# nintendops/EPN_PointCloud

Measured on AMD Instinct MI355X. Metric: point-clouds/sec fwd+bwd, ModelNet40 N=1024 A=60, higher is better.
Workload: dtype f32

## Files before the change

epn_pointcloud_amd/csrc/c_api.hip:

```cpp
#include <atomic>
#include <cstdlib>
#include <cstring>
#include <cxxabi.h>

#include "conv_internal.h"

using namespace epn;

static std::atomic<int> g_policy{0};
static bool force_generic() { return g_policy.load(std::memory_order_relaxed) == 1; }

namespace epn {
bool first_layer_on_valu() { return g_policy.load(std::memory_order_relaxed) == 2; }
#ifdef EPN_TUNING
int kernel_policy() { return g_policy.load(std::memory_order_relaxed); }
#else
int kernel_policy() { return 0; }
#endif
}

namespace {
thread_local const void *t_stub = nullptr;
thread_local bool t_stub_aux = true;
}
namespace epn {
void note_kernel(const void *host_stub, bool aux) {
    if (aux && t_stub) return;
    t_stub = host_stub;
    t_stub_aux = aux;
}
}

extern "C" const char *epn_last_kernel(void) {
    static thread_local char out[320];
    out[0] = 0;
    const void *stub = t_stub;
    t_stub = nullptr;
    t_stub_aux = true;
    if (!stub) return out;
    const char *mangled = hipKernelNameRefByPtr(stub, nullptr);
    if (!mangled) return out;
    int status = 0;
    char *dem = abi::__cxa_demangle(mangled, nullptr, nullptr, &status);
    const char *b = (status == 0 && dem) ? dem : mangled;
    if (!std::strncmp(b, "void ", 5)) b += 5;
    static const char anon[] = "(anonymous namespace)::";
    size_t o = 0;
    int depth = 0;
    for (size_t i = 0; b[i] && o + 1 < sizeof(out);) {
        if (!std::strncmp(b + i, anon, sizeof(anon) - 1)) { i += sizeof(anon) - 1; continue; }
        if (b[i] == '<') ++depth;
        else if (b[i] == '>') --depth;
        else if (b[i] == '(' && depth == 0) break;
        out[o++] = b[i++];
    }
    out[o] = 0;
    std::free(dem);
    return out;
}

extern "C" int epn_set_kernel_policy(int policy) {
#ifdef EPN_TUNING
    if (policy != 0 && policy != 1 && policy != 2 && (policy & ~0xff) != 0x100 && (policy & ~0xff) != 0x200 && (policy & ~0xff) != 0x400 && (policy & ~0xff) != 0x800 && (policy & ~0xff) != 0x900) return EPN_EINVAL;
#else
    if (policy != 0 && policy != 1 && policy != 2) return EPN_EINVAL;
#endif
    g_policy.store(policy, std::memory_order_relaxed);
    return 0;
}

static int check_desc(const epn_inter_desc *d) {
    if (!d) return EPN_ENULL;
    if (d->b < 0 || d->p1 < 1 || d->p2 < 0 || d->nn < 1 || d->na < 1 || d->ks < 1 || d->cin < 1 || d->cout < 1)
        return EPN_EINVAL;
    if (d->ks > EPN_KS_GENERIC_MAX) return EPN_EINVAL;
    if (!(d->sigma > 0.f) && !d->dense_w) return EPN_EINVAL;
    if (!d->ball_idx) return EPN_ENULL;
    if (!d->dense_w && (!d->xyz || !d->new_xyz || !d->anchors || !d->kernels)) return EPN_ENULL;
    return 0;
}

static bool use_mfma(const epn_inter_desc *d) { return inter_uses_mfma(d) && !force_generic() && !d->dense_w; }

extern "C" const char *epn_version(void) { return "epn_so3conv 0.5 (gfx950)"; }
extern "C" int epn_abi_version(void) { return EPN_ABI_VERSION; }

extern "C" const char *epn_strerror(int code) {
    switch (code) {
        case 0: return "success";
        case EPN_EINVAL: return "epn: invalid size or unsupported shape";
        case EPN_EWORKSPACE: return "epn: workspace missing or too small";
        case EPN_ENULL: return "epn: required pointer is NULL";
        default: return code > 0 ? hipGetErrorString((hipError_t)code) : "epn: unknown error";
    }
}

extern "C" int epn_inter_is_fused(const epn_inter_desc *d) {
    return d && (use_mfma(d) || (inter_c1_fwd_ok(d) && !force_generic())) ? 1 : 0;
}

extern "C" int epn_intra_is_fused(int na, int kn, int cin, int cout) {
    return intra_uses_mfma(na, kn, cin, cout) && !force_generic() ? 1 : 0;
}

extern "C" size_t epn_inter_workspace_bytes(const epn_inter_desc *d) {
    if (!d) return 0;
    InterWs w = inter_ws(d);
    if (force_generic() || d->dense_w) {
        epn_inter_desc g = *d;
        g.cin = d->cin; g.cout = d->cout;
        const size_t big = (size_t)d->b * d->p2 * d->na * d->cin * d->ks;
        return (w.big_off + rnd64(big)) * sizeof(float);
    }
    return w.total_floats * sizeof(float);
}

static int prep(const epn_inter_desc *d, void *workspace, size_t bytes, bool need_big, InterWs &ws, float *&base,
                hipStream_t st, bool need_rk = true) {
    int rc = check_desc(d);
    if (rc) return rc;
    ws = inter_ws(d);
    const size_t big = need_big ? rnd64((size_t)d->b * d->p2 * d->na * d->cin * d->ks)
                                : ws.total_floats - ws.big_off;
    if (!workspace || bytes < (ws.big_off + big) * sizeof(float)) return EPN_EWORKSPACE;
    base = static_cast<float *>(workspace);
    if (!d->dense_w && need_rk) {
        rc = launch_rk_table(d, base + ws.rk_off, st);
        if (rc) return rc;
    }
    return 0;
}

extern "C" int epn_inter_weights_f32(const epn_inter_desc *d, float *w, epn_stream_t stream) {
    int rc = check_desc(d);
    if (rc) return rc;
    if (!w || !d->xyz || !d->new_xyz || !d->anchors || !d->kernels) return EPN_ENULL;
    if (d->b == 0 || d->p2 == 0) return 0;
    return launch_inter_weights(d, w, epn_stream(stream));
}

extern "C" int epn_inter_so3conv_fwd_f32(const epn_inter_desc *d, const float *feats_cl, const float *W,
                                         float *out_cl, void *workspace, size_t workspace_bytes,
                                         epn_stream_t stream) {
    hipStream_t st = epn_stream(stream);
    InterWs ws;
    float *base = nullptr;
    const bool mf = d && use_mfma(d);
    int rc = prep(d, workspace, workspace_bytes, !mf, ws, base, st, !mf);
// ... 431 lines not shown
```

epn_pointcloud_amd/csrc/gemm.h:

```cpp
#pragma once
#include "epn_common.h"

namespace epn {

constexpr int GEMM_MAX_PROB = 6;

struct GemmNtProb {
    const void *A, *Bt;
    void *C;
    long long M, lda, ldb, ldc;
    int N, K;
    int tiles_n;
    unsigned tile0;
    unsigned ntile;
    const void *Bp;
    float *stats;
    const float *a_amax, *b_amax;
    unsigned *c_amax;
};
struct GemmNtBatch {
    int nprob;
    unsigned ntiles;
    GemmNtProb p[GEMM_MAX_PROB];
};
// ... 131 lines not shown
    mfma_term(acc, al, bh);
    mfma_term(acc, am, bm);
    mfma_term(acc, ah, bm);
    mfma_term(acc, am, bh);
    mfma_term(acc, ah, bh);
}
template <int TM, int TN>
__device__ __forceinline__ void f2_terms(gemm_f32x16 (&acc)[TM][TN], const gemm_f16x8 (&ah)[TM], const gemm_f16x8 (&al)[TM],
                                         const gemm_f16x8 (&bh)[TN], const gemm_f16x8 (&bl)[TN]) {
    mfma_term(acc, ah, bl);
    mfma_term(acc, al, bh);
    mfma_term(acc, ah, bh);
}
template <int TM, int TN>
__device__ __forceinline__ float f2_unscale(gemm_f32x16 (&acc)[TM][TN], float ux, float uy) {
    float chk = 0.0f;
#pragma unroll
    for (int i = 0; i < TM; ++i)
#pragma unroll
        for (int j = 0; j < TN; ++j)
#pragma unroll
            for (int r = 0; r < 16; ++r) {
                chk = fmaf(acc[i][j][r], 0.0f, chk);
                acc[i][j][r] = acc[i][j][r] * ux * uy;
            }
    return chk;
}

template <int TM, int TN, typename TO>
__device__ __forceinline__ void nt_col_stats(const gemm_f32x16 (&acc)[TM][TN], float *__restrict__ part, long long M, int N,
                                             long long row0, int col0, int li, int lj) {
#pragma unroll
    for (int i = 0; i < TM; ++i) {
        const long long rb = row0 + 32 * i;
        if (rb >= M) continue;
#pragma unroll
        for (int j = 0; j < TN; ++j) {
            float s1 = 0.f, s2 = 0.f;
#pragma unroll
            for (int r = 0; r < 16; ++r) {
                float v = acc[i][j][r];
                if constexpr (sizeof(TO) == 2) v = (float)(__bf16)v;
                s1 += v;
                s2 = fmaf(v, v, s2);
            }
            s1 += __shfl_xor(s1, 32, 64);
            s2 += __shfl_xor(s2, 32, 64);
            const int n = col0 + 32 * j + li;
            if (lj == 0 && n < N) {
                float2 *o = reinterpret_cast<float2 *>(part + (((size_t)(rb >> 5)) * N + n) * 2);
                *o = make_float2(s1, s2);
            }
        }
    }
}
#endif

#ifdef __HIPCC__
template <int TM, int TN, typename TO>
__device__ __forceinline__ void nt_c_amax(const gemm_f32x16 (&acc)[TM][TN], unsigned *__restrict__ out) {
    float mf = 0.0f;
#pragma unroll
    for (int i = 0; i < TM; ++i)
#pragma unroll
        for (int j = 0; j < TN; ++j)
#pragma unroll
            for (int r = 0; r < 16; r += 2) mf = fmaxf(fmaxf(mf, fabsf(acc[i][j][r])), fabsf(acc[i][j][r + 1]));
    if constexpr (sizeof(TO) == 2) mf = (float)(__bf16)mf;
    unsigned m = __builtin_bit_cast(unsigned, mf);
    m = m < 0x7f800000u ? m : 0u;
#pragma unroll
    for (int o = 32; o >= 1; o >>= 1) {
        const unsigned v = (unsigned)__shfl_xor((int)m, o, 64);
        m = v > m ? v : m;
    }
    if ((threadIdx.x & 63) == 0 && m > __atomic_load_n(out, __ATOMIC_RELAXED)) atomicMax(out, m);
}
#endif

long long f2_nonfinite_take_gemm(bool reset);
long long f2_nonfinite_take_x3(bool reset);
long long f2_nonfinite_take_bwd(bool reset);

int kernel_policy();

int launch_gemm_nt(GemmNtBatch &B, int dtype, int out_dtype, hipStream_t st);
bool gemm_nt_x3_ok(const GemmNtBatch &B);
size_t gemm_nt_x3_workspace(const GemmNtBatch &B);
int launch_gemm_nt_x3(GemmNtBatch &B, void *ws, size_t ws_bytes, hipStream_t st, int npl = 3);
size_t gemm_nt_f2_workspace(const GemmNtBatch &B);
int launch_absmax(const float *src, long long ld, long long rows, long long cols, float *out, hipStream_t st);
int launch_scale_scalar(float *v, float factor, hipStream_t st, unsigned tag = 0);
int launch_absmax_unless_tagged(const float *src, long long n, float *slot, unsigned tag, hipStream_t st);
int launch_gemm_tn(GemmTnArgs &G, int dtype, hipStream_t st);
int launch_gemm_tn_batch(GemmTnBatch &B, int dtype, void *ws, size_t ws_bytes, hipStream_t st);
size_t gemm_tn_batch_workspace(GemmTnBatch &B, int dtype);
void gemm_tn_tile(int dtype, int N1, int N2, int *bn1, int *bn2);
int gemm_tn_splits(int dtype, long long R, int N1, int N2);
int launch_transpose_cast(const void *src, void *dst, int rows, int cols, int src_bf16, int dst_bf16, hipStream_t st);
int launch_cast(const void *src, void *dst, size_t n, int src_bf16, int dst_bf16, hipStream_t st);
int launch_cast_add(const float *src, const void *add_bf16, void *dst_bf16, size_t n, hipStream_t st);

}
```

epn_pointcloud_amd/csrc/gemm_tn.hip:

```cpp
#include "conv_internal.h"
#include "gemm.h"

namespace epn {
namespace {
EPN_F2_SENTINEL_DECL


#ifndef EPN_TN_GROUP_TARGET_BF16
#define EPN_TN_GROUP_TARGET_BF16 768
#endif
#ifndef EPN_TN_GROUP_TARGET_F32
#define EPN_TN_GROUP_TARGET_F32 1024
#endif
#ifndef EPN_TN_SINGLE_TARGET_BF16
#define EPN_TN_SINGLE_TARGET_BF16 512
#endif
#ifndef EPN_TN_SWZ
#define EPN_TN_SWZ 1
#endif
__device__ __forceinline__ int tn_row_swz(int r) { return 2 * ((r & 3) | (((r >> 3) & 1) << 2)); }
template <bool SWZ>
__device__ __forceinline__ int tn_swz_col(int col, int r) {
    if constexpr (!SWZ) return col;
    return (((col >> 3) ^ tn_row_swz(r)) << 3) | (col & 7);
}
#ifndef EPN_TN_WIDE_NSTG
#define EPN_TN_WIDE_NSTG 3
#endif
#ifndef EPN_TN_NARROW_NSTG
#define EPN_TN_NARROW_NSTG 4
#endif
#ifndef EPN_TN_NARROW_STAGE_KB
#define EPN_TN_NARROW_STAGE_KB 32
#endif
constexpr int tn_ring_kr(int wgm, int wgn, int tm, int tn) {
    const int step_b = 32 * 2 * 16 * (wgm * tm + wgn * tn);
    int kr = 1;
    while (2 * kr * step_b <= EPN_TN_NARROW_STAGE_KB * 1024 && 2 * kr * step_b * EPN_TN_NARROW_NSTG <= 160 * 1024) kr *= 2;
    return kr;
}
#ifndef EPN_TN_NARROW_WGS
#define EPN_TN_NARROW_WGS 1
#endif
__device__ __forceinline__ unsigned tn_tile_of(unsigned lb, unsigned ntiles, unsigned nsplit) {
    return epn_xcd_tile(lb, (ntiles * nsplit + 7u) & ~7u);
}

template <int W, int K>
__device__ __forceinline__ void tn_frag_k(const char *p, float (&v)[W][K], int k) {
    static_assert(W == 1 || W == 2 || W == 4, "fragment width");
    if constexpr (W == 4) {
        const f32x4 q = *reinterpret_cast<const f32x4 *>(p);
        v[0][k] = q[0]; v[1][k] = q[1]; v[2][k] = q[2]; v[3][k] = q[3];
    } else if constexpr (W == 2) {
        const f32x2 q = *reinterpret_cast<const f32x2 *>(p);
        v[0][k] = q[0]; v[1][k] = q[1];
    } else {
        v[0][k] = *reinterpret_cast<const float *>(p);
    }
}
template <int W>
__device__ __forceinline__ void tn_frag(const char *p, float (&v)[W]) {
    static_assert(W == 1 || W == 2 || W == 4, "fragment width");
    if constexpr (W == 4) {
        const f32x4 q = *reinterpret_cast<const f32x4 *>(p);
        v[0] = q[0]; v[1] = q[1]; v[2] = q[2]; v[3] = q[3];
    } else if constexpr (W == 2) {
        const f32x2 q = *reinterpret_cast<const f32x2 *>(p);
        v[0] = q[0]; v[1] = q[1];
    } else {
        v[0] = *reinterpret_cast<const float *>(p);
    }
}

template <int WGM, int WGN, int TM, int TN, int BR, int X3 = 0>
__global__ __launch_bounds__(64 * WGM * WGN) void gemm_tn_f32_kernel(GemmTnBatch B) {
    constexpr int NW = WGM * WGN;
    constexpr int BN1 = WGM * TM * 32, BN2 = WGN * TN * 32;
    constexpr int ROWF = BN1 + BN2;
    constexpr int STAGE_B = BR * ROWF * 4;
    constexpr int NI = STAGE_B / 1024;
    constexpr int IPW = (NI + NW - 1) / NW;
    static_assert(STAGE_B % 1024 == 0, "stage must be a whole number of 1 KiB pieces");
    __shared__ __attribute__((aligned(1024))) char smem[2 * STAGE_B];

    const int lane = threadIdx.x & 63;
    const int wave = __builtin_amdgcn_readfirstlane(threadIdx.x >> 6);
    int pi = 0;
#pragma unroll
    for (int i = 1; i < GEMM_MAX_PROB; ++i)
        if (i < B.nprob && blockIdx.x >= B.p[i].block0) pi = i;
    const GemmTnArgs &G = B.p[pi];
    const unsigned tile = tn_tile_of(blockIdx.x - G.block0, G.ntiles, (unsigned)G.nsplit) % G.ntiles;
    const unsigned split = tn_tile_of(blockIdx.x - G.block0, G.ntiles, (unsigned)G.nsplit) / G.ntiles;
    if (split >= (unsigned)G.nsplit) return;
    const int n1_0 = (int)(tile / G.tiles_n2) * BN1, n2_0 = (int)(tile % G.tiles_n2) * BN2;
    const long long nchunk = G.R / BR;
    const long long c0 = nchunk * split / G.nsplit, c1 = nchunk * (split + 1) / G.nsplit;
    const int nk = (int)(c1 - c0);
    const float *__restrict__ X = static_cast<const float *>(G.X);
    const float *__restrict__ Y = static_cast<const float *>(G.Y);

    const float *src[IPW];
    long long sstep[IPW];
#pragma unroll
    for (int i = 0; i < IPW; ++i) {
        const int q = wave + i * NW;
        const int fo = 256 * q + 4 * lane;
        const int r = fo / ROWF, c = fo % ROWF;
        if (c < BN1) {
            int n = n1_0 + c;
            n = n < G.N1 - 4 ? n : G.N1 - 4;
            src[i] = X + (c0 * BR + r) * G.ldx + n;
            sstep[i] = (long long)BR * G.ldx;
        } else {
            int n = n2_0 + (c - BN1);
            n = n < G.N2 - 4 ? n : G.N2 - 4;
            src[i] = Y + (c0 * BR + r) * G.ldy + n;
            sstep[i] = (long long)BR * G.ldy;
        }
    }
    auto stage_one = [&](int buf, int i) {
        const int q = wave + i * NW;
// ... 515 lines not shown
            src[i] += sstep[i];
        }
    };

    const int wm = wave / WGN, wn = wave % WGN;
    const int li = lane & 15, lg = lane >> 4;
    const int tr_row = 8 * lg + (li >> 2), tr_col = 4 * (li & 3);

    f32x4 acc[TM][TN];
#pragma unroll
    for (int i = 0; i < TM; ++i)
#pragma unroll
        for (int j = 0; j < TN; ++j) acc[i][j] = f32x4{0.f, 0.f, 0.f, 0.f};

#pragma unroll
    for (int s = 0; s < NSTG - 1; ++s)
        if (s < nst) stage(s);
    typedef short s16x8 __attribute__((ext_vector_type(8)));
    for (int kt = 0; kt < nst; ++kt) {
        const int ahead = nst - 1 - kt;
        if (NSTG == 4 && ahead >= 2) asm volatile("s_waitcnt vmcnt(%0)" ::"n"(2 * IPW) : "memory");
        else if (ahead >= 1) asm volatile("s_waitcnt vmcnt(%0)" ::"n"(IPW) : "memory");
        else asm volatile("s_waitcnt vmcnt(0)" ::: "memory");
        __builtin_amdgcn_s_barrier();
        asm volatile("" ::: "memory");
        const char *sbase = smem + (kt % NSTG) * STAGE_B;
#pragma unroll
        for (int ks = 0; ks < KR; ++ks) {
            if (KR > 1 && kt * KR + ks >= nk) break;
            const char *base = sbase + ks * (32 * ROWE * 2);
            s16x4 lo[TM + TN], hi[TM + TN];
#pragma unroll
            for (int f = 0; f < TM + TN; ++f) {
                const int col = tn_swz_col<SWZ>(f < TN ? BN1 + (wn * TN + f) * 16 + tr_col : (wm * TM + (f - TN)) * 16 + tr_col, tr_row);
                const unsigned ad =
                    (unsigned)(uintptr_t)(__attribute__((address_space(3))) char *)(base + (tr_row * ROWE + col) * 2);
                asm volatile("ds_read_b64_tr_b16 %0, %1" : "=v"(lo[f]) : "v"(ad));
                asm volatile("ds_read_b64_tr_b16 %0, %1 offset:%2" : "=v"(hi[f]) : "v"(ad), "n"(4 * ROWE * 2));
            }
            bf16x8 b[TN];
#pragma unroll
            for (int i = 0; i < TM; ++i) {
                asm volatile("s_waitcnt lgkmcnt(%0)" ::"n"(2 * (TM - 1 - i)) : "memory");
                if (i == 0) {
#pragma unroll
                    for (int j = 0; j < TN; ++j) {
                        asm volatile("" : "+v"(lo[j]), "+v"(hi[j]));
                        const s16x8 v = {lo[j][0], lo[j][1], lo[j][2], lo[j][3], hi[j][0], hi[j][1], hi[j][2], hi[j][3]};
                        b[j] = __builtin_bit_cast(bf16x8, v);
                    }
                }
                asm volatile("" : "+v"(lo[TN + i]), "+v"(hi[TN + i]));
                const s16x8 va = {lo[TN + i][0], lo[TN + i][1], lo[TN + i][2], lo[TN + i][3],
                                  hi[TN + i][0], hi[TN + i][1], hi[TN + i][2], hi[TN + i][3]};
                const bf16x8 a = __builtin_bit_cast(bf16x8, va);
#pragma unroll
                for (int j = 0; j < TN; ++j) {
                    acc[i][j] = __builtin_amdgcn_mfma_f32_16x16x32_bf16(a, b[j], acc[i][j], 0, 0, 0);
                    if (ks == 0 && i == 0 && j == 0) {
                        __builtin_amdgcn_sched_barrier(0);
                        if (kt + NSTG - 1 < nst) stage((kt + NSTG - 1) % NSTG);
                        __builtin_amdgcn_sched_barrier(0);
                    }
                }
            }
        }
    }

    float *__restrict__ C = G.nsplit > 1 ? static_cast<float *>(G.part) + (size_t)split * G.N1 * G.N2
                                         : static_cast<float *>(G.C);
    const long long ldc = G.nsplit > 1 ? G.N2 : G.ldc;
#pragma unroll
    for (int i = 0; i < TM; ++i)
#pragma unroll
        for (int j = 0; j < TN; ++j)
#pragma unroll
            for (int r = 0; r < 4; ++r) {
                const int n1 = n1_0 + (wm * TM + i) * 16 + 4 * lg + r;
                const int n2 = n2_0 + (wn * TN + j) * 16 + li;
                if (n1 < G.N1 && n2 < G.N2) C[(long long)n1 * ldc + n2] = acc[i][j][r];
            }
}

__global__ __launch_bounds__(256) void gemm_tn_reduce_kernel(GemmTnBatch B) {
    const GemmTnArgs &G = B.p[blockIdx.y];
    if (G.nsplit <= 1) return;
    const float *__restrict__ part = static_cast<const float *>(G.part);
    float *__restrict__ C = static_cast<float *>(G.C);
    const size_t n = (size_t)G.N1 * G.N2;
    const size_t stride = (size_t)gridDim.x * blockDim.x;
    if ((G.N2 & 3) == 0 && (G.ldc & 3) == 0 && !((uintptr_t)C & 15)) {
        const size_t n4 = n >> 2;
        for (size_t i = (size_t)blockIdx.x * blockDim.x + threadIdx.x; i < n4; i += stride) {
            const f32x4 *p = reinterpret_cast<const f32x4 *>(part) + i;
            f32x4 a[8];
#pragma unroll
            for (int u = 0; u < 8; ++u) a[u] = f32x4{0.f, 0.f, 0.f, 0.f};
            int k = 0;
            for (; k + 8 <= G.nsplit; k += 8)
#pragma unroll
                for (int u = 0; u < 8; ++u) {
                    const f32x4 v = p[(size_t)(k + u) * n4];
                    a[u][0] += v[0]; a[u][1] += v[1]; a[u][2] += v[2]; a[u][3] += v[3];
                }
            for (; k < G.nsplit; ++k) {
                const f32x4 v = p[(size_t)k * n4];
                a[0][0] += v[0]; a[0][1] += v[1]; a[0][2] += v[2]; a[0][3] += v[3];
            }
            f32x4 r;
#pragma unroll
            for (int e = 0; e < 4; ++e)
                r[e] = ((a[0][e] + a[1][e]) + (a[2][e] + a[3][e])) + ((a[4][e] + a[5][e]) + (a[6][e] + a[7][e]));
            const size_t e0 = i << 2;
            *reinterpret_cast<f32x4 *>(C + (e0 / G.N2) * G.ldc + (e0 % G.N2)) = r;
        }
        return;
    }
    for (size_t i = (size_t)blockIdx.x * blockDim.x + threadIdx.x; i < n; i += stride) {
        float s = 0.f;
        for (int k = 0; k < G.nsplit; ++k) s += part[(size_t)k * n + i];
        C[(i / G.N2) * G.ldc + (i % G.N2)] = s;
    }
}

template <int SP>
__global__ __launch_bounds__(256) void gemm_tn_reduce_sp_kernel(GemmTnBatch B) {
    constexpr int QB = 256 / SP;
    __shared__ f32x4 red[SP][QB];
    const GemmTnArgs &G = B.p[blockIdx.y];
    if (G.nsplit <= 1) return;
    const f32x4 *__restrict__ part = static_cast<const f32x4 *>(G.part);
    float *__restrict__ C = static_cast<float *>(G.C);
    const size_t n4 = ((size_t)G.N1 * G.N2) >> 2;
    const int ql = threadIdx.x % QB, g = threadIdx.x / QB;
    for (size_t q0 = (size_t)blockIdx.x * QB; q0 < n4; q0 += (size_t)gridDim.x * QB) {
        const size_t q = q0 + ql;
        f32x4 a[4];
#pragma unroll
        for (int u = 0; u < 4; ++u) a[u] = f32x4{0.f, 0.f, 0.f, 0.f};
        if (q < n4) {
            int k = g;
            for (; k + 3 * SP < G.nsplit; k += 4 * SP)
#pragma unroll
                for (int u = 0; u < 4; ++u) {
                    const f32x4 v = part[(size_t)(k + u * SP) * n4 + q];
                    a[u][0] += v[0]; a[u][1] += v[1]; a[u][2] += v[2]; a[u][3] += v[3];
                }
            for (; k < G.nsplit; k += SP) {
                const f32x4 v = part[(size_t)k * n4 + q];
                a[0][0] += v[0]; a[0][1] += v[1]; a[0][2] += v[2]; a[0][3] += v[3];
            }
        }
        f32x4 r;
#pragma unroll
        for (int e = 0; e < 4; ++e) r[e] = (a[0][e] + a[1][e]) + (a[2][e] + a[3][e]);
        red[g][ql] = r;
        __syncthreads();
        if (g == 0 && q < n4) {
            for (int j = 1; j < SP; ++j) {
                const f32x4 v = red[j][ql];
                r[0] += v[0]; r[1] += v[1]; r[2] += v[2]; r[3] += v[3];
            }
            const size_t e0 = q << 2;
            *reinterpret_cast<f32x4 *>(C + (e0 / G.N2) * G.ldc + (e0 % G.N2)) = r;
        }
        __syncthreads();
    }
}

template <typename T>
__global__ void gemm_tn_generic_kernel(const T *__restrict__ X, const T *__restrict__ Y, float *__restrict__ C,
                                       long long R, int N1, int N2, long long ldx, long long ldy, long long ldc) {
    const long long i = (long long)blockIdx.x * blockDim.x + threadIdx.x;
    if (i >= (long long)N1 * N2) return;
    const int n1 = (int)(i / N2), n2 = (int)(i % N2);
    float s = 0.f;
    for (long long r = 0; r < R; ++r) s = fmaf((float)X[r * ldx + n1], (float)Y[r * ldy + n2], s);
    C[(long long)n1 * ldc + n2] = s;
}

enum TnFamily { TN_F32, TN_PLANES, TN_BF16, TN_RING };
#define EPN_TN_F32_INSTANCES(X)                                                                                      \
    X(1, 8, 1, 2, 32)                                                                                 \
    X(2, 2, 1, 1, 32)                                                                                 \
    X(2, 2, 1, 2, 32)                                                                                 \
    X(1, 8, 2, 1, 32)                                                                                 \
    X(1, 4, 2, 4, 16)                                                                                 \
    X(2, 2, 2, 1, 32)                                                                                 \
    X(2, 2, 2, 2, 32)                                                                                 \
    X(2, 4, 2, 2, 32)                                                                                 \
    X(1, 8, 4, 2, 32)
#define EPN_TN_PLANES_INSTANCES(X)                                                                                   \
    X(1, 8, 1, 2, 32)                                                                                 \
    X(1, 8, 2, 2, 16)                                                                                 \
    X(2, 4, 2, 2, 32)                                   \
    X(1, 8, 4, 2, 16)                                                                                 \
    X(2, 4, 4, 2, 16)
#define EPN_TN_BF16_INSTANCES(X)                                                                                     \
    X(1, 4, 2, 4)                                                                                     \
    X(1, 4, 4, 4)                                                                                     \
    X(2, 2, 4, 8)
#define EPN_TN_RING_NARROW(X, TM, TN) X(2, 2, TM, TN, EPN_TN_NARROW_NSTG, tn_ring_kr(2, 2, TM, TN))
#define EPN_TN_RING_INSTANCES(X)                                                                                     \
    EPN_TN_RING_NARROW(X, 1, 1)                                                                       \
    EPN_TN_RING_NARROW(X, 2, 1)                                                                       \
    EPN_TN_RING_NARROW(X, 1, 2)                                                                       \
    EPN_TN_RING_NARROW(X, 2, 2)                                                                       \
    EPN_TN_RING_NARROW(X, 4, 2)                                                                       \
    EPN_TN_RING_NARROW(X, 8, 2)                                                                       \
    EPN_TN_RING_NARROW(X, 1, 4)                                                                       \
    EPN_TN_RING_NARROW(X, 2, 4)                                                                       \
    EPN_TN_RING_NARROW(X, 4, 4)                                                                       \
    EPN_TN_RING_NARROW(X, 8, 4)                                                                       \
    X(2, 2, 4, 8, EPN_TN_WIDE_NSTG, 1)

struct TnChoice {
    TnFamily family;
    int bn1, bn2;
    bool planes;
    size_t ws_bytes;
    size_t amax_off;
};

inline bool tn_has_instance(TnFamily f, int bn1, int bn2) {
#define EPN_TN_IS32(WGM, WGN, TM, TN, ...) || (bn1 == WGM * TM * 32 && bn2 == WGN * TN * 32)
#define EPN_TN_IS16(WGM, WGN, TM, TN, ...) || (bn1 == WGM * TM * 16 && bn2 == WGN * TN * 16)
    switch (f) {
        case TN_F32: return false EPN_TN_F32_INSTANCES(EPN_TN_IS32);
        case TN_PLANES: return false EPN_TN_PLANES_INSTANCES(EPN_TN_IS32);
        case TN_BF16: return false EPN_TN_BF16_INSTANCES(EPN_TN_IS16);
        case TN_RING: return false EPN_TN_RING_INSTANCES(EPN_TN_IS16);
    }
#undef EPN_TN_IS32
#undef EPN_TN_IS16
    return false;
}

template <typename T>
int launch_tn_instance(const TnChoice &ch, const GemmTnBatch &B, hipStream_t st, int x3) {
    const dim3 grid(B.nblocks);
#define EPN_TN_F32(WGM, WGN, TM, TN, BR)                                                                                       \
    if (ch.bn1 == WGM * TM * 32 && ch.bn2 == WGN * TN * 32) {                                                                  \
        if (x3 == 3) EPN_LAUNCH((gemm_tn_f32_kernel<WGM, WGN, TM, TN, BR, 3>), grid, dim3(64 * WGM * WGN), 0, st, B);          \
        else if (x3 == 2) EPN_LAUNCH((gemm_tn_f32_kernel<WGM, WGN, TM, TN, BR, 2>), grid, dim3(64 * WGM * WGN), 0, st, B);     \
        else EPN_LAUNCH((gemm_tn_f32_kernel<WGM, WGN, TM, TN, BR, 0>), grid, dim3(64 * WGM * WGN), 0, st, B);                  \
        return 0;                                                                                                              \
    }
#define EPN_TN_PLANES(WGM, WGN, TM, TN, BR)                                                                                    \
    if (ch.bn1 == WGM * TM * 32 && ch.bn2 == WGN * TN * 32) {                                                                  \
        if (x3 == 3) EPN_LAUNCH((gemm_tn_x3_kernel<WGM, WGN, TM, TN, BR, 3>), grid, dim3(64 * WGM * WGN), 0, st, B);           \
        else EPN_LAUNCH((gemm_tn_x3_kernel<WGM, WGN, TM, TN, BR, 2>), grid, dim3(64 * WGM * WGN), 0, st, B);                   \
        return 0;                                                                                                              \
    }
#define EPN_TN_BF16(WGM, WGN, TM, TN)                                                                                          \
    if (ch.bn1 == WGM * TM * 16 && ch.bn2 == WGN * TN * 16) {                                                                  \
        EPN_LAUNCH((gemm_tn_bf16_kernel<WGM, WGN, TM, TN>), grid, dim3(64 * WGM * WGN), 0, st, B);                             \
        return 0;                                                                                                              \
    }
#define EPN_TN_RING(WGM, WGN, TM, TN, NSTG, KR)                                                                                \
    if (ch.bn1 == WGM * TM * 16 && ch.bn2 == WGN * TN * 16) {                                                                  \
        EPN_LAUNCH((gemm_tn_bf16_ring_kernel<WGM, WGN, TM, TN, NSTG, KR>), grid, dim3(64 * WGM * WGN), 0, st, B);              \
        return 0;                                                                                                              \
    }
    if constexpr (sizeof(T) == 4) {
        if (ch.family == TN_F32) { EPN_TN_F32_INSTANCES(EPN_TN_F32) }
        if (ch.family == TN_PLANES) { EPN_TN_PLANES_INSTANCES(EPN_TN_PLANES) }
    } else {
        if (ch.family == TN_BF16) { EPN_TN_BF16_INSTANCES(EPN_TN_BF16) }
        if (ch.family == TN_RING) { EPN_TN_RING_INSTANCES(EPN_TN_RING) }
    }
#undef EPN_TN_F32
#undef EPN_TN_PLANES
#undef EPN_TN_BF16
#undef EPN_TN_RING
    return EPN_EINVAL;
}

#ifndef EPN_TN_GROUP_PLANES
#define EPN_TN_GROUP_PLANES 512
#endif
inline int tn_group_planes(int x3) { return x3 == 2 ? EPN_TN_GROUP_PLANES / 2 : EPN_TN_GROUP_PLANES; }
inline bool tn_planes_form(int nprob, int N2, int x3) { return N2 >= (nprob == 1 ? 512 : tn_group_planes(x3)); }

template <typename T>
bool tn_fast_ok(const GemmTnArgs &G) {
    constexpr int E16 = ElemOf<T>::PER16;
    return G.R > 0 && G.R % 32 == 0 && G.N1 >= E16 && G.N2 >= E16 && G.ldx % E16 == 0 && G.ldy % E16 == 0 &&
           !((uintptr_t)G.X & 15) && !((uintptr_t)G.Y & 15) && G.N1 % E16 == 0 && G.N2 % E16 == 0;
}

template <typename T>
TnChoice tn_plan(GemmTnBatch &B, void *ws, int x3 = 0) {
    const int bf = sizeof(T) == 2 ? 1 : (x3 ? 2 : 0);
    int max1 = 0, min2 = 1 << 30;
    for (int i = 0; i < B.nprob; ++i) {
        max1 = B.p[i].N1 > max1 ? B.p[i].N1 : max1;
        min2 = B.p[i].N2 < min2 ? B.p[i].N2 : min2;
    }
    int bn1, bn2;
    gemm_tn_tile(B.nprob > 1 && bf == 2 ? 0 : bf, max1, B.nprob > 1 && min2 < 256 ? 256 : min2, &bn1, &bn2);
    if (B.nprob > 1 && bf == 2 && min2 >= tn_group_planes(x3)) {
        int min1 = 1 << 30;
        for (int i = 0; i < B.nprob; ++i) min1 = B.p[i].N1 < min1 ? B.p[i].N1 : min1;
        if (min1 >= 256) { bn1 = 256; bn2 = 256; }
    }
    if (B.nprob > 1 && x3 == 2 && min2 < 256) { bn1 = 128; bn2 = 128; }
    long long tiles[GEMM_MAX_PROB], chunks[GEMM_MAX_PROB];
    for (int i = 0; i < B.nprob; ++i) {
        GemmTnArgs &G = B.p[i];
        G.tiles_n2 = (G.N2 + bn2 - 1) / bn2;
        G.ntiles = (unsigned)((G.N1 + bn1 - 1) / bn1) * G.tiles_n2;
        tiles[i] = G.ntiles;
        chunks[i] = G.R / 32;
    }
    if (B.nprob == 1) {
        B.p[0].nsplit = gemm_tn_splits(bf, B.p[0].R, B.p[0].N1, B.p[0].N2);
    } else {
        const long long target = bf == 1 ? EPN_TN_GROUP_TARGET_BF16 : EPN_TN_GROUP_TARGET_F32;
        long long S = 8;
        for (long long cand = 8; cand <= 8192; ++cand) {
            long long blocks = 0;
            for (int i = 0; i < B.nprob; ++i) blocks += tiles[i] * ((chunks[i] + cand - 1) / cand);
            S = cand;
            if (blocks <= target) break;
        }
        for (int i = 0; i < B.nprob; ++i) {
            long long sp = (chunks[i] + S - 1) / S;
            sp = sp < 1 ? 1 : (sp > 512 ? 512 : sp);
            B.p[i].nsplit = (int)sp;
        }
    }
    size_t off = 0;
    unsigned blk = 0;
    for (int i = 0; i < B.nprob; ++i) {
        GemmTnArgs &G = B.p[i];
        G.block0 = blk;
        blk += (G.ntiles * (unsigned)G.nsplit + 7u) & ~7u;
        G.part = nullptr; G.part_bytes = 0;
        if (G.nsplit > 1) {
            const size_t nb = (size_t)G.nsplit * G.N1 * G.N2 * sizeof(float);
            if (ws) G.part = static_cast<char *>(ws) + off;
            G.part_bytes = nb;
            off += (nb + 255) & ~(size_t)255;
        }
    }
    B.nblocks = blk;
    for (int i = 0; i < B.nprob; ++i) B.p[i].Xp = nullptr;
    const bool planes = x3 && tn_has_instance(TN_PLANES, bn1, bn2) && tn_planes_form(B.nprob, min2, x3);
    if (planes)
        for (int i = 0; i < B.nprob; ++i) {
            GemmTnArgs &G = B.p[i];
            G.Xp = ws ? static_cast<char *>(ws) + off : reinterpret_cast<const void *>(1);
            off += ((size_t)2 * x3 * G.R * G.N1 + 255) & ~(size_t)255;
        }
    size_t amax_off = 0;
    if (x3 == 2) {
        amax_off = off;
        off += 256;
    }
    TnFamily family = planes ? TN_PLANES : TN_F32;
    if constexpr (sizeof(T) == 2) family = (B.nprob == 1 ? bn2 <= 128 : bn1 == 128) ? TN_RING : TN_BF16;
    return TnChoice{family, bn1, bn2, planes, off, amax_off};
}

template <typename T>
int launch_tn_typed(GemmTnBatch &B, void *ws, size_t ws_bytes, hipStream_t st, int x3 = 0) {
    bool fast = true;
    for (int i = 0; i < B.nprob; ++i) {
        const GemmTnArgs &G = B.p[i];
        if (G.R < 0 || G.N1 < 1 || G.N2 < 1) return EPN_EINVAL;
        if (!G.C) return EPN_ENULL;
        if (G.R > 0 && (!G.X || !G.Y)) return EPN_ENULL;
        fast = fast && tn_fast_ok<T>(G);
    }
    if (!fast) {
        for (int i = 0; i < B.nprob; ++i) {
            const GemmTnArgs &G = B.p[i];
            const long long n = (long long)G.N1 * G.N2;
            EPN_LAUNCH((gemm_tn_generic_kernel<T>), dim3((unsigned)((n + 255) / 256)), dim3(256), 0, st,
                               static_cast<const T *>(G.X), static_cast<const T *>(G.Y), static_cast<float *>(G.C), G.R,
                               G.N1, G.N2, G.ldx, G.ldy, G.ldc);
            EPN_CHECK_LAUNCH();
        }
        return 0;
    }
    const TnChoice ch = tn_plan<T>(B, ws, x3);
    if (ch.ws_bytes > 0 && (!ws || ws_bytes < ch.ws_bytes)) return EPN_EWORKSPACE;
    if (!tn_has_instance(ch.family, ch.bn1, ch.bn2)) return EPN_EINVAL;
    if constexpr (sizeof(T) == 4) {
        if (x3 == 2) {
            float *slots = reinterpret_cast<float *>(static_cast<char *>(ws) + ch.amax_off);
            for (int i = 0; i < B.nprob; ++i) {
                GemmTnArgs &G = B.p[i];
                if (!G.x_amax) {
                    int rc = launch_absmax(static_cast<const float *>(G.X), G.ldx, G.R, G.N1, slots + 2 * i, st);
                    if (rc) return rc;
                    G.x_amax = slots + 2 * i;
                }
                if (!G.y_amax) {
                    int rc = launch_absmax(static_cast<const float *>(G.Y), G.ldy, G.R, G.N2, slots + 2 * i + 1, st);
                    if (rc) return rc;
                    G.y_amax = slots + 2 * i + 1;
                }
            }
        }
        if (ch.planes) {
            for (int i = 0; i < B.nprob; ++i) {
                const GemmTnArgs &G = B.p[i];
                const long long n = (G.R >> 3) * G.N1;
                if (x3 == 3)
                    EPN_LAUNCH_AUX(split_octets_kernel, dim3((unsigned)((n + 255) / 256)), dim3(256), 0, st,
                                   static_cast<const float *>(G.X), G.ldx, G.R, G.N1, static_cast<u32x4 *>(const_cast<void *>(G.Xp)));
                else
                    EPN_LAUNCH_AUX(split_octets2_kernel, dim3((unsigned)((n + 255) / 256)), dim3(256), 0, st,
                                   static_cast<const float *>(G.X), G.ldx, G.R, G.N1, static_cast<u32x4 *>(const_cast<void *>(G.Xp)), G.x_amax);
                EPN_CHECK_LAUNCH();
            }
        }
    }
    const int rc = launch_tn_instance<T>(ch, B, st, x3);
    if (rc) return rc;
    EPN_CHECK_LAUNCH();
    bool any_split = false;
    size_t nmax = 0;
    for (int i = 0; i < B.nprob; ++i) {
        any_split = any_split || B.p[i].nsplit > 1;
        const size_t n = (size_t)B.p[i].N1 * B.p[i].N2;
        nmax = n > nmax ? n : nmax;
    }
    if (any_split) {
        const size_t nv = (nmax + 3) / 4;
        bool quads = true;
        int smax = 1;
        for (int i = 0; i < B.nprob; ++i) {
            const GemmTnArgs &G = B.p[i];
            quads = quads && (G.N2 & 3) == 0 && (G.ldc & 3) == 0 && !((uintptr_t)G.C & 15);
            smax = G.nsplit > smax ? G.nsplit : smax;
        }
        int sp = 1;
        while (quads && sp < 64 && smax > 16 * sp && nv * B.nprob * sp * 4 <= (1u << 20)) sp *= 4;
        if (sp > 1) {
            const size_t qb = 256 / sp;
            const unsigned gx = (unsigned)((nv + qb - 1) / qb < 2048 ? (nv + qb - 1) / qb : 2048);
// ... 158 lines not shown
```

Measured before the change: 539.6.

## Add multi-stage LDS ring kernel for f32 split-precision TN GEMM

Adds a new f32 TN GEMM kernel for the x3==2 split-precision path. It streams X and Y rows into a 3- or 4-stage LDS ring using direct global-to-LDS loads and explicit vmcnt waits, then reads fragments with raw ds_read, splits them into hi/lo f16 and accumulates with MFMA. The planner selects it by default whenever the non-planes path has a matching tile instance, and policy 3 restores the old two-stage kernel. The aim is to overlap global loads with compute and cut synchronisation stalls, at the cost of more LDS per block and hand-written waitcnt logic that could hide ordering bugs.

```diff
diff --git a/epn_pointcloud_amd/csrc/c_api.hip b/epn_pointcloud_amd/csrc/c_api.hip
--- a/epn_pointcloud_amd/csrc/c_api.hip
+++ b/epn_pointcloud_amd/csrc/c_api.hip
@@ -12,6 +12,7 @@
 
 namespace epn {
 bool first_layer_on_valu() { return g_policy.load(std::memory_order_relaxed) == 2; }
+bool tn_f32_two_stage() { return g_policy.load(std::memory_order_relaxed) == 3; }
 #ifdef EPN_TUNING
 int kernel_policy() { return g_policy.load(std::memory_order_relaxed); }
 #else
@@ -61,9 +62,9 @@
 
 extern "C" int epn_set_kernel_policy(int policy) {
 #ifdef EPN_TUNING
-    if (policy != 0 && policy != 1 && policy != 2 && (policy & ~0xff) != 0x100 && (policy & ~0xff) != 0x200 && (policy & ~0xff) != 0x400 && (policy & ~0xff) != 0x800 && (policy & ~0xff) != 0x900) return EPN_EINVAL;
+    if (policy != 0 && policy != 1 && policy != 2 && policy != 3 && (policy & ~0xff) != 0x100 && (policy & ~0xff) != 0x200 && (policy & ~0xff) != 0x400 && (policy & ~0xff) != 0x800 && (policy & ~0xff) != 0x900) return EPN_EINVAL;
 #else
-    if (policy != 0 && policy != 1 && policy != 2) return EPN_EINVAL;
+    if (policy != 0 && policy != 1 && policy != 2 && policy != 3) return EPN_EINVAL;
 #endif
     g_policy.store(policy, std::memory_order_relaxed);
     return 0;
diff --git a/epn_pointcloud_amd/csrc/gemm.h b/epn_pointcloud_amd/csrc/gemm.h
--- a/epn_pointcloud_amd/csrc/gemm.h
+++ b/epn_pointcloud_amd/csrc/gemm.h
@@ -237,6 +237,7 @@
 long long f2_nonfinite_take_x3(bool reset);
 long long f2_nonfinite_take_bwd(bool reset);
 
+bool tn_f32_two_stage();
 int kernel_policy();
 
 int launch_gemm_nt(GemmNtBatch &B, int dtype, int out_dtype, hipStream_t st);
diff --git a/epn_pointcloud_amd/csrc/gemm_tn.hip b/epn_pointcloud_amd/csrc/gemm_tn.hip
--- a/epn_pointcloud_amd/csrc/gemm_tn.hip
+++ b/epn_pointcloud_amd/csrc/gemm_tn.hip
@@ -1,3 +1,5 @@
+#include <type_traits>
+
 #include "conv_internal.h"
 #include "gemm.h"
 
@@ -33,12 +35,24 @@
 #ifndef EPN_TN_NARROW_STAGE_KB
 #define EPN_TN_NARROW_STAGE_KB 32
 #endif
+constexpr int tn_ring_kr_of(int step_b, int nstg) {
+    int kr = 1;
+    while (2 * kr * step_b <= EPN_TN_NARROW_STAGE_KB * 1024 && 2 * kr * step_b * nstg <= 160 * 1024) kr *= 2;
+    return kr;
+}
 constexpr int tn_ring_kr(int wgm, int wgn, int tm, int tn) {
-    const int step_b = 32 * 2 * 16 * (wgm * tm + wgn * tn);
-    int kr = 1;
-    while (2 * kr * step_b <= EPN_TN_NARROW_STAGE_KB * 1024 && 2 * kr * step_b * EPN_TN_NARROW_NSTG <= 160 * 1024) kr *= 2;
-    return kr;
-}
+    return tn_ring_kr_of(32 * 2 * 16 * (wgm * tm + wgn * tn), EPN_TN_NARROW_NSTG);
+}
+constexpr int tn_f32_ring_step_b(int wgm, int wgn, int tm, int tn) { return 32 * 4 * 32 * (wgm * tm + wgn * tn); }
+constexpr int tn_f32_ring_nstg(int wgm, int wgn, int tm, int tn) {
+    return 4 * tn_f32_ring_step_b(wgm, wgn, tm, tn) <= 160 * 1024 ? 4 : 3;
+}
+constexpr int tn_f32_ring_kr(int wgm, int wgn, int tm, int tn) {
+    return tn_ring_kr_of(tn_f32_ring_step_b(wgm, wgn, tm, tn), tn_f32_ring_nstg(wgm, wgn, tm, tn));
+}
+#ifndef EPN_TN_F32_RING
+#define EPN_TN_F32_RING 1
+#endif
 #ifndef EPN_TN_NARROW_WGS
 #define EPN_TN_NARROW_WGS 1
 #endif
@@ -720,6 +734,184 @@
             }
 }
 
+template <int W> struct TnFragVec;
+template <> struct TnFragVec<1> { typedef float type; };
+template <> struct TnFragVec<2> { typedef f32x2 type; };
+template <int N, typename Fn>
+__device__ __forceinline__ void tn_static_for(Fn &&f) {
+    if constexpr (N > 0) {
+        tn_static_for<N - 1>(f);
+        f(std::integral_constant<int, N - 1>{});
+    }
+}
+template <int W, int OFF>
+__device__ __forceinline__ void tn_lds_read(unsigned ad, typename TnFragVec<W>::type &v) {
+    static_assert(OFF >= 0 && OFF < 65536, "ds offset field");
+    if constexpr (W == 2) asm volatile("ds_read_b64 %0, %1 offset:%2" : "=v"(v) : "v"(ad), "n"(OFF));
+    else asm volatile("ds_read_b32 %0, %1 offset:%2" : "=v"(v) : "v"(ad), "n"(OFF));
+}
+template <int W>
+__device__ __forceinline__ void tn_frag_unpack(typename TnFragVec<W>::type (&raw)[8], float (&v)[W][8]) {
+#pragma unroll
+    for (int k = 0; k < 8; ++k) {
+        asm volatile("" : "+v"(raw[k]));
+        if constexpr (W == 2) { v[0][k] = raw[k][0]; v[1][k] = raw[k][1]; }
+        else v[0][k] = raw[k];
+    }
+}
+
+template <int WGM, int WGN, int TM, int TN, int NSTG, int KR>
+__global__ __launch_bounds__(64 * WGM * WGN) void gemm_tn_f32_ring_kernel(GemmTnBatch B) {
+    constexpr int NW = WGM * WGN;
+    constexpr int BN1 = WGM * TM * 32, BN2 = WGN * TN * 32;
+    constexpr int ROWF = BN1 + BN2;
+    constexpr int ROWB = ROWF * 4;
+    constexpr int BR = 32 * KR;
+    constexpr int STAGE_B = BR * ROWB;
+    constexpr int NI = STAGE_B / 1024;
+    constexpr int IPW = (NI + NW - 1) / NW;
+    static_assert(TM <= 2 && TN <= 2, "fragment reads of 4 or 8 bytes (conflict-free in the linear image)");
+    static_assert(STAGE_B % 1024 == 0, "stage must be a whole number of 1 KiB pieces");
+    static_assert(NSTG >= 3 && NSTG <= 4 && NSTG * STAGE_B <= 160 * 1024, "ring of 3 or 4 stages in LDS");
+    static_assert(IPW * (NSTG - 2) <= 63, "vmcnt range");
+    __shared__ __attribute__((aligned(1024))) char smem[NSTG * STAGE_B];
+
+    const int lane = threadIdx.x & 63;
+    const int wave = __builtin_amdgcn_readfirstlane(threadIdx.x >> 6);
+    int pi = 0;
+#pragma unroll
+    for (int i = 1; i < GEMM_MAX_PROB; ++i)
+        if (i < B.nprob && blockIdx.x >= B.p[i].block0) pi = i;
+    const GemmTnArgs &G = B.p[pi];
+    const unsigned tile = tn_tile_of(blockIdx.x - G.block0, G.ntiles, (unsigned)G.nsplit) % G.ntiles;
+    const unsigned split = tn_tile_of(blockIdx.x - G.block0, G.ntiles, (unsigned)G.nsplit) / G.ntiles;
+    if (split >= (unsigned)G.nsplit) return;
+    const int n1_0 = (int)(tile / G.tiles_n2) * BN1, n2_0 = (int)(tile % G.tiles_n2) * BN2;
+    const long long nchunk = G.R / 32;
+    const long long c0 = nchunk * split / G.nsplit, c1 = nchunk * (split + 1) / G.nsplit;
+    const int nk = (int)(c1 - c0);
+    const int nst = (nk + KR - 1) / KR;
+    const float *__restrict__ X = static_cast<const float *>(G.X);
+    const float *__restrict__ Y = static_cast<const float *>(G.Y);
+
+    float x_scale = f2_scale_of(*G.x_amax), y_scale = f2_scale_of(*G.y_amax);
+    asm volatile("" : "+v"(x_scale), "+v"(y_scale));
+
+    const float *src[IPW], *lim[IPW];
+    long long sstep[IPW];
+#pragma unroll
+    for (int i = 0; i < IPW; ++i) {
+        const int q = (wave + i * NW) % NI;
+        const int fo = 256 * q + 4 * lane;
+        const int r = fo / ROWF, c = fo % ROWF;
+        if (c < BN1) {
+            int n = n1_0 + c;
+            n = n < G.N1 - 4 ? n : G.N1 - 4;
+            src[i] = X + (c0 * 32 + r) * G.ldx + n;
+            lim[i] = X + (G.R - 1) * G.ldx + n;
+            sstep[i] = (long long)BR * G.ldx;
+        } else {
+            int n = n2_0 + (c - BN1);
+            n = n < G.N2 - 4 ? n : G.N2 - 4;
+            src[i] = Y + (c0 * 32 + r) * G.ldy + n;
+            lim[i] = Y + (G.R - 1) * G.ldy + n;
+            sstep[i] = (long long)BR * G.ldy;
+        }
+    }
+    auto stage = [&](int buf) {
+#pragma unroll
+        for (int i = 0; i < IPW; ++i) {
+            const int q = (wave + i * NW) % NI;
+            glds16(KR > 1 && src[i] > lim[i] ? lim[i] : src[i], smem + buf * STAGE_B + q * 1024);
+            src[i] += sstep[i];
+        }
+    };
+
+    const int wm = wave / WGN, wn = wave % WGN;
+    const int li = lane & 31, lj = lane >> 5;
+    const unsigned lds0 = (unsigned)(uintptr_t)(__attribute__((address_space(3))) char *)smem + 8 * lj * ROWB;
+    const unsigned xad0 = lds0 + (wm * TM * 32 + TM * li) * 4;
+    const unsigned yad0 = lds0 + (BN1 + wn * TN * 32 + TN * li) * 4;
+
+    f32x16 acc[TM][TN];
+#pragma unroll
+    for (int i = 0; i < TM; ++i)
+#pragma unroll
+        for (int j = 0; j < TN; ++j)
+#pragma unroll
+            for (int r = 0; r < 16; ++r) acc[i][j][r] = 0.f;
+
+#pragma unroll
+    for (int s = 0; s < NSTG - 1; ++s)
+        if (s < nst) stage(s);
+    for (int kt = 0; kt < nst; ++kt) {
+        const int ahead = nst - 1 - kt;
+        if (NSTG == 4 && ahead >= 2) asm volatile("s_waitcnt vmcnt(%0)" ::"n"(2 * IPW) : "memory");
+        else if (ahead >= 1) asm volatile("s_waitcnt vmcnt(%0)" ::"n"(IPW) : "memory");
+        else asm volatile("s_waitcnt vmcnt(0)" ::: "memory");
+        __builtin_amdgcn_s_barrier();
+        asm volatile("" ::: "memory");
+        if (kt + NSTG - 1 < nst) stage((kt + NSTG - 1) % NSTG);
+        const unsigned sb = (unsigned)(kt % NSTG) * STAGE_B;
+        const unsigned xad = xad0 + sb, yad = yad0 + sb;
+        const int left = nk - kt * KR;
+        tn_static_for<2 * KR>([&](auto F) {
+            constexpr int f = decltype(F)::value;
+            if (KR > 1 && f / 2 >= left) return;
+            typename TnFragVec<TM>::type xr[8];
+            typename TnFragVec<TN>::type yr[8];
+            tn_static_for<8>([&](auto K) {
+                constexpr int off = (16 * f + decltype(K)::value) * ROWB;
+                tn_lds_read<TM, off>(xad, xr[decltype(K)::value]);
+                tn_lds_read<TN, off>(yad, yr[decltype(K)::value]);
+            });
+            asm volatile("s_waitcnt lgkmcnt(0)" ::: "memory");
+            float xa[TM][8], yb[TN][8];
+            tn_frag_unpack<TM>(xr, xa);
+            tn_frag_unpack<TN>(yr, yb);
+            gemm_f16x8 ah[TM], al[TM], bh[TN], bl[TN];
+#pragma unroll
+            for (int i = 0; i < TM; ++i) f2_split8(xa[i], x_scale, ah[i], al[i]);
+#pragma unroll
+            for (int j = 0; j < TN; ++j) f2_split8(yb[j], y_scale, bh[j], bl[j]);
+            f2_terms(acc, ah, al, bh, bl);
+        });
+    }
+
+    const float ux = f2_inverse(x_scale), uy = f2_inverse(y_scale);
+    EPN_F2_CHECK(f2_unscale(acc, ux, uy));
+    float *__restrict__ C = G.nsplit > 1 ? static_cast<float *>(G.part) + (size_t)split * G.N1 * G.N2
+                                         : static_cast<float *>(G.C);
+    const long long ldc = G.nsplit > 1 ? G.N2 : G.ldc;
+    if (n1_0 + BN1 <= G.N1 && n2_0 + BN2 <= G.N2 && (long long)BN1 * ldc < (1LL << 30)) {
+        float *__restrict__ cw = C + (size_t)(n1_0 + wm * TM * 32) * ldc + (n2_0 + wn * TN * 32);
+        const unsigned ld = (unsigned)ldc;
+        const unsigned lane_off = (unsigned)(TM * 4 * lj) * ld + TN * li;
+#pragma unroll
+        for (int i = 0; i < TM; ++i)
+#pragma unroll
+            for (int r = 0; r < 16; ++r) {
+                const unsigned o = lane_off + (unsigned)(TM * ((r & 3) + 8 * (r >> 2)) + i) * ld;
+#pragma unroll
+                for (int j = 0; j < TN; ++j) cw[o + j] = acc[i][j][r];
+            }
+        return;
+    }
+#pragma unroll
+    for (int i = 0; i < TM; ++i)
+#pragma unroll
+        for (int r = 0; r < 16; ++r) {
+            const int ri = (r & 3) + 8 * (r >> 2) + 4 * lj;
+            const int n1 = n1_0 + wm * TM * 32 + TM * ri + i;
+            const int n2 = n2_0 + wn * TN * 32 + TN * li;
+            if (n1 < G.N1) {
+#pragma unroll
+                for (int j = 0; j < TN; ++j)
+                    if (n2 + j < G.N2) C[(long long)n1 * ldc + n2 + j] = acc[i][j][r];
+            }
+        }
+}
+
 __global__ __launch_bounds__(256) void gemm_tn_reduce_kernel(GemmTnBatch B) {
     const GemmTnArgs &G = B.p[blockIdx.y];
     if (G.nsplit <= 1) return;
@@ -817,7 +1009,7 @@
     C[(long long)n1 * ldc + n2] = s;
 }
 
-enum TnFamily { TN_F32, TN_PLANES, TN_BF16, TN_RING };
+enum TnFamily { TN_F32, TN_PLANES, TN_BF16, TN_RING, TN_F32_RING };
 #define EPN_TN_F32_INSTANCES(X)                                                                                      \
     X(1, 8, 1, 2, 32)                                                                                 \
     X(2, 2, 1, 1, 32)                                                                                 \
@@ -852,6 +1044,15 @@
     EPN_TN_RING_NARROW(X, 8, 4)                                                                       \
     X(2, 2, 4, 8, EPN_TN_WIDE_NSTG, 1)
 
+#define EPN_TN_F32_RING_ONE(X, WGM, WGN, TM, TN)                                                                     \
+    X(WGM, WGN, TM, TN, tn_f32_ring_nstg(WGM, WGN, TM, TN), tn_f32_ring_kr(WGM, WGN, TM, TN))
+#define EPN_TN_F32_RING_INSTANCES(X)                                                                                 \
+    EPN_TN_F32_RING_ONE(X, 2, 2, 1, 1)                                   \
+    EPN_TN_F32_RING_ONE(X, 2, 2, 1, 2)                                   \
+    EPN_TN_F32_RING_ONE(X, 2, 2, 2, 1)                                   \
+    EPN_TN_F32_RING_ONE(X, 2, 2, 2, 2)                                   \
+    EPN_TN_F32_RING_ONE(X, 2, 4, 2, 2)
+
 struct TnChoice {
     TnFamily family;
     int bn1, bn2;
@@ -868,6 +1069,7 @@
         case TN_PLANES: return false EPN_TN_PLANES_INSTANCES(EPN_TN_IS32);
         case TN_BF16: return false EPN_TN_BF16_INSTANCES(EPN_TN_IS16);
         case TN_RING: return false EPN_TN_RING_INSTANCES(EPN_TN_IS16);
+        case TN_F32_RING: return false EPN_TN_F32_RING_INSTANCES(EPN_TN_IS32);
     }
 #undef EPN_TN_IS32
 #undef EPN_TN_IS16
@@ -900,7 +1102,13 @@
         EPN_LAUNCH((gemm_tn_bf16_ring_kernel<WGM, WGN, TM, TN, NSTG, KR>), grid, dim3(64 * WGM * WGN), 0, st, B);              \
         return 0;                                                                                                              \
     }
+#define EPN_TN_F32_RING_L(WGM, WGN, TM, TN, NSTG, KR)                                                                          \
+    if (ch.bn1 == WGM * TM * 32 && ch.bn2 == WGN * TN * 32) {                                                                  \
+        EPN_LAUNCH((gemm_tn_f32_ring_kernel<WGM, WGN, TM, TN, NSTG, KR>), grid, dim3(64 * WGM * WGN), 0, st, B);               \
+        return 0;                                                                                                              \
+    }
     if constexpr (sizeof(T) == 4) {
+        if (ch.family == TN_F32_RING && x3 == 2) { EPN_TN_F32_RING_INSTANCES(EPN_TN_F32_RING_L) }
         if (ch.family == TN_F32) { EPN_TN_F32_INSTANCES(EPN_TN_F32) }
         if (ch.family == TN_PLANES) { EPN_TN_PLANES_INSTANCES(EPN_TN_PLANES) }
     } else {
@@ -911,6 +1119,7 @@
 #undef EPN_TN_PLANES
 #undef EPN_TN_BF16
 #undef EPN_TN_RING
+#undef EPN_TN_F32_RING_L
     return EPN_EINVAL;
 }
 
@@ -997,6 +1206,8 @@
         off += 256;
     }
     TnFamily family = planes ? TN_PLANES : TN_F32;
+    if (EPN_TN_F32_RING && x3 == 2 && !planes && !tn_f32_two_stage() && tn_has_instance(TN_F32_RING, bn1, bn2))
+        family = TN_F32_RING;
     if constexpr (sizeof(T) == 2) family = (B.nprob == 1 ? bn2 <= 128 : bn1 == 128) ? TN_RING : TN_BF16;
     return TnChoice{family, bn1, bn2, planes, off, amax_off};
 }
```

Result: slower. 533.5 (-1.1%).
